# Themaister/Granite

Measured on AMD Instinct MI355X. Metric: Mpixels/s for clustered-light+post chain @4K; achieved HBM GB/s vs roofline, higher is better.
Workload: dtype f32

## Files before the change

### granite_amd/csrc/cluster.hip

```cpp
#include "ctx.hpp"
#include "device_common.hpp"
#include "device_vec.hpp"

namespace
{
__device__ __forceinline__ v4 mul_mat4(const float *m, v4 v)
{
	v4 r = mk4(m[0], m[1], m[2], m[3]) * v.x;
	r = r + mk4(m[4], m[5], m[6], m[7]) * v.y;
	r = r + mk4(m[8], m[9], m[10], m[11]) * v.z;
	r = r + mk4(m[12], m[13], m[14], m[15]) * v.w;
	return r;
}

__device__ __forceinline__ float min_tie2(float a, float b) { return a < b ? a : b; }
__device__ __forceinline__ float max_tie2(float a, float b) { return a > b ? a : b; }

struct TransformedSpot { v4 clip[5]; v4 z; };
struct CullSetup { v4 data[32]; };

__device__ __forceinline__ const gr_light_info *lights_of(const void *transforms)
{
	return reinterpret_cast<const gr_light_info *>(static_cast<const uint8_t *>(transforms) + GR_TRANSFORMS_OFFSET_LIGHTS);
}
// ... 111 lines not shown
	bool dual;
	switch (code)
	{
	case 1u: a = c0; b = c1; c = c2; dual = true; break;
	case 2u: a = c1; b = c2; c = c0; dual = true; break;
	case 4u: a = c2; b = c0; c = c1; dual = true; break;
	case 3u: a = c0; b = c1; c = c2; dual = false; break;
	case 5u: a = c2; b = c0; c = c1; dual = false; break;
	default: a = c1; b = c2; c = c0; dual = false; break;
	}
	const float target = 0.0f;
	if (dual)
	{
		const float l_ab = (target - a.z) / (b.z - a.z);
		const float l_ac = (target - a.z) / (c.z - a.z);
		const v3 ab = mix3(a, b, l_ab);
		const v3 ac = mix3(a, c, l_ac);
		emit_triangle(cs, num_triangles, Tri2{{xy(ab), xy(b), xy(ac)}}, cull);
		emit_triangle(cs, num_triangles, Tri2{{xy(ac), xy(b), xy(c)}}, cull);
	}
	else
	{
		const float la = (target - a.z) / (c.z - a.z);
		const float lb = (target - b.z) / (c.z - b.z);
		a = mix3(a, c, la);
		b = mix3(b, c, lb);
		emit_triangle(cs, num_triangles, Tri2{{xy(a), xy(b), xy(c)}}, cull);
	}
}

__device__ void clip_w_and_project(CullSetup &cs, uint32_t &num_triangles, v4 c0, v4 c1, v4 c2, float cull)
{
	const float MIN_W = 1.0f / 1024.0f;
	const uint32_t code = uint32_t(c0.w < MIN_W) + uint32_t(c1.w < MIN_W) * 2u + uint32_t(c2.w < MIN_W) * 4u;
	if (code == 7u)
		return;
	if (code == 0u)
	{
		clip_near_z(cs, num_triangles, Tri3{{xyz(c0) / c0.w, xyz(c1) / c1.w, xyz(c2) / c2.w}}, cull);
		return;
	}
	v4 a, b, c;
	bool dual;
	switch (code)
	{
	case 1u: a = c0; b = c1; c = c2; dual = true; break;
	case 2u: a = c1; b = c2; c = c0; dual = true; break;
	case 4u: a = c2; b = c0; c = c1; dual = true; break;
	case 3u: a = c0; b = c1; c = c2; dual = false; break;
	case 5u: a = c2; b = c0; c = c1; dual = false; break;
	default: a = c1; b = c2; c = c0; dual = false; break;
	}
	if (dual)
	{
		const float l_ab = (MIN_W - a.w) / (b.w - a.w);
		const float l_ac = (MIN_W - a.w) / (c.w - a.w);
		const v4 ab = mix4(a, b, l_ab);
		const v4 ac = mix4(a, c, l_ac);
		clip_near_z(cs, num_triangles, Tri3{{xyz(ab) / MIN_W, xyz(b) / b.w, xyz(ac) / MIN_W}}, cull);
		clip_near_z(cs, num_triangles, Tri3{{xyz(ac) / MIN_W, xyz(b) / b.w, xyz(c) / c.w}}, cull);
	}
	else
	{
		const float la = (MIN_W - a.w) / (c.w - a.w);
		const float lb = (MIN_W - b.w) / (c.w - b.w);
		a = mix4(a, c, la);
		b = mix4(b, c, lb);
		clip_near_z(cs, num_triangles, Tri3{{xyz(a) / MIN_W, xyz(b) / MIN_W, xyz(c) / c.w}}, cull);
	}
}

__device__ __forceinline__ void cluster_setup_of(bool point, const gr_light_info &li, const TransformedSpot &spot, CullSetup &cs,
                                                 const gr_cluster_params &params, const gr_push_cluster_setup &push)
{
	if (point)
	{
		const float radius = 1.0f / li.inv_radius;
		const v4 v4d = mul_mat4(push.view, mk4(li.position[0], li.position[1], li.position[2], 1.0f));
		const v3 view = mk3(v4d.x, -v4d.y, -v4d.z);
		const v2 r0 = project_sphere_flat(view.x, view.z, radius);
		const v2 r1 = project_sphere_flat(view.y, view.z, radius);
		const float xy_length = len2(mk2(view.x, view.y));
		v2 ct0, ct1;
		if (xy_length < 0.00001f)
		{
			ct0 = mk2(1.0f, 0.0f);
			ct1 = mk2(0.0f, 1.0f);
		}
		else
		{
			const float inv_xy_length = 1.0f / xy_length;
			ct0 = mk2(view.x, -view.y) * inv_xy_length;
			ct1 = mk2(view.y, view.x) * inv_xy_length;
		}
		const v2 txy = mk2(ct0.x * view.x + ct1.x * view.y, ct0.y * view.x + ct1.y * view.y);
		const v2 t0 = project_sphere_flat(txy.x, view.z, radius);
		const v2 t1 = project_sphere_flat(txy.y, view.z, radius);
		const bool ellipsis = !isinf(t0.x) && !isinf(t0.y) && !isinf(t1.x) && !isinf(t1.y);
		const v2 center = (mk2(t0.x, t1.x) + mk2(t0.y, t1.y)) * 0.5f;
		const v2 ellipse_radius = mk2(t0.y, t1.y) - center;
		cs.data[0] = mk4(r0.x * params.clip_scale[0], r1.x * params.clip_scale[1], r0.y * params.clip_scale[0],
		                 r1.y * params.clip_scale[1]);
		cs.data[1] = mk4(t0.x, t0.y, t1.x, t1.y);
		cs.data[2] = mk4(ct0.x, ct0.y, ct1.x, ct1.y);
		cs.data[3] = mk4(ellipsis ? 1.0f : 0.0f, 1.0f / ellipse_radius.x, 1.0f / ellipse_radius.y, 0.0f);
	}
	else
	{
		const v4 z = spot.z;
		if (z.x != 0.0f)
		{
			uint32_t n = 0u;
			const v4 c0 = spot.clip[0], c1 = spot.clip[1], c2 = spot.clip[2];
			const v4 c3 = spot.clip[3], c4 = spot.clip[4];
			clip_w_and_project(cs, n, c0, c1, c2, z.x);
			clip_w_and_project(cs, n, c0, c2, c3, z.x);
			clip_w_and_project(cs, n, c0, c3, c4, z.x);
			clip_w_and_project(cs, n, c0, c4, c1, z.x);
			clip_w_and_project(cs, n, c2, c1, c3, z.x);
			clip_w_and_project(cs, n, c4, c3, c1, z.x);
			cs.data[0].w = __uint_as_float(n);
		}
		else
			cs.data[0].w = __uint_as_float(0xffffffffu);
	}
}

__global__ __launch_bounds__(64) void k_cluster_setup(const void *transforms, const TransformedSpot *spots, CullSetup *setup,
                                                      gr_cluster_params params, gr_push_cluster_setup push)
{
	const uint32_t index = blockIdx.x * 64u + threadIdx.x;
	if (index >= push.num_lights)
		return;
	const bool point = (type_mask_of(transforms)[index >> 5u] & (1u << (index & 31u))) != 0u;
	cluster_setup_of(point, lights_of(transforms)[index], spots[index], setup[index], params, push);
}

__device__ bool test_point_light(const gr_cluster_params &prm, const CullSetup &cs, v2 uv, v2 uv_stride)
{
	const v4 eir = cs.data[3];
	if (eir.x != 0.0f)
	{
		const v4 tr = cs.data[1];
		const v4 ct = cs.data[2];
		const v2 center = (mk2(tr.x, tr.z) + mk2(tr.y, tr.w)) * 0.5f;
		const v2 cszw = mk2(prm.clip_scale[2], prm.clip_scale[3]);
		const v2 lo = uv * cszw;
		const v2 hi = (uv + uv_stride) * cszw;
		const v2 inv_r = mk2(eir.y, eir.z);
		const v2 d00 = (mk2(ct.x * lo.x + ct.z * lo.y, ct.y * lo.x + ct.w * lo.y) - center) * inv_r;
		const v2 d01 = (mk2(ct.x * lo.x + ct.z * hi.y, ct.y * lo.x + ct.w * hi.y) - center) * inv_r;
		const v2 d10 = (mk2(ct.x * hi.x + ct.z * lo.y, ct.y * hi.x + ct.w * lo.y) - center) * inv_r;
		const v2 d11 = (mk2(ct.x * hi.x + ct.z * hi.y, ct.y * hi.x + ct.w * hi.y) - center) * inv_r;
		const float max_diag = fmaxf(dist2(d00, d11), dist2(d01, d10));
		float min_sq_dist = 1.0f + max_diag;
		min_sq_dist *= min_sq_dist;
		return dot2(d00, d00) < min_sq_dist && dot2(d01, d01) < min_sq_dist && dot2(d10, d10) < min_sq_dist &&
		       dot2(d11, d11) < min_sq_dist;
	}
	const v4 bb = cs.data[0];
	const v2 hi = uv + uv_stride;
	return hi.x > bb.x && hi.y > bb.y && uv.x < bb.z && uv.y < bb.w;
}

__device__ bool test_spot_light(const CullSetup &cs, v2 uv, v2 uv_stride)
{
	const uint32_t num_triangles = __float_as_uint(cs.data[0].w);
	if (num_triangles > 8u)
		return true;
	const v2 hi = uv + uv_stride;
	for (uint32_t i = 0; i < num_triangles; i++)
	{
		const v4 bb = cs.data[4u * i + 3u];
		if (hi.x > bb.x && hi.y > bb.y && uv.x < bb.z && uv.y < bb.w)
		{
			v3 base = xyz(cs.data[4u * i]);
			const v3 dx = xyz(cs.data[4u * i + 1u]);
			const v3 dy = xyz(cs.data[4u * i + 2u]);
			base = base + dx * uv.x;
			base = base + dy * uv.y;
			base = base + mk3(dx.x > 0.0f ? uv_stride.x * dx.x : 0.0f, dx.y > 0.0f ? uv_stride.x * dx.y : 0.0f,
			                  dx.z > 0.0f ? uv_stride.x * dx.z : 0.0f);
			base = base + mk3(dy.x > 0.0f ? uv_stride.y * dy.x : 0.0f, dy.y > 0.0f ? uv_stride.y * dy.y : 0.0f,
			                  dy.z > 0.0f ? uv_stride.y * dy.z : 0.0f);
			if (base.x > 0.0f && base.y > 0.0f && base.z > 0.0f)
				return true;
		}
	}
	return false;
}

__global__ __launch_bounds__(64) void k_cluster_binning(const void *transforms, const CullSetup *setup, uint32_t *bitmask,
                                                        gr_cluster_params prm)
{
	const uint32_t lane = threadIdx.x;
	const uint32_t chunk = blockIdx.x;
	const uint32_t tile_x = blockIdx.y, tile_y = blockIdx.z;
	const v2 inv_res = mk2(prm.inv_resolution_xy[0], prm.inv_resolution_xy[1]);
	const uint32_t type_mask = type_mask_of(transforms)[chunk];

	const v2 tile_uv = mk2(2.0f * float(tile_x * 8u), 2.0f * float(tile_y * 8u)) * inv_res - mk2(1.0f, 1.0f);
	const v2 tile_stride = mk2(2.0f * 8.0f, 2.0f * 8.0f) * inv_res;

	bool passed = false;
	if (lane < 32u)
	{
		const uint32_t light_index = 32u * chunk + lane;
		if (light_index < uint32_t(prm.num_lights))
		{
			if ((type_mask >> lane) & 1u)
				passed = test_point_light(prm, setup[light_index], tile_uv, tile_stride);
			else
				passed = test_spot_light(setup[light_index], tile_uv, tile_stride);
		}
	}
	uint32_t ballot = uint32_t(__ballot(passed));

	const uint32_t px = tile_x * 8u + (lane & 7u), py = tile_y * 8u + (lane >> 3u);
	const v2 uv = mk2(2.0f * float(px), 2.0f * float(py)) * inv_res - mk2(1.0f, 1.0f);
	const v2 uv_stride = inv_res * 2.0f;
	uint32_t pixel_mask = 0u;
	while (ballot != 0u)
	{
		const int lsb = __builtin_ctz(ballot);
		ballot &= ballot - 1u;
		const uint32_t light_index = chunk * 32u + uint32_t(lsb);
		bool hit;
		if ((type_mask >> lsb) & 1u)
			hit = test_point_light(prm, setup[light_index], uv, uv_stride);
		else
			hit = test_spot_light(setup[light_index], uv, uv_stride);
		if (hit)
			pixel_mask |= 1u << lsb;
	}
	const uint32_t linear_coord = py * uint32_t(prm.resolution_xy[0]) + px;
	bitmask[size_t(linear_coord) * uint32_t(prm.num_lights_32) + chunk] = pixel_mask;
}

constexpr int ZR_THREADS = 256;
constexpr int ZR_SLICES_PER_WAVE = 4;
constexpr int ZR_SLICES = (ZR_THREADS / 64) * ZR_SLICES_PER_WAVE;

__device__ __forceinline__ uint32_t zr_wave_min(uint32_t v)
{
#pragma unroll
	for (int off = 32; off > 0; off >>= 1)
		v = min(v, uint32_t(__shfl_xor(int(v), off, 64)));
	return v;
}
__device__ __forceinline__ uint32_t zr_wave_max(uint32_t v)
{
#pragma unroll
	for (int off = 32; off > 0; off >>= 1)
		v = max(v, uint32_t(__shfl_xor(int(v), off, 64)));
	return v;
}

__device__ __forceinline__ void z_range_block(const uint2 *light_ranges, uint2 *out, const gr_push_z_range &push, uint32_t slice_block, uint8_t *smem,
                                              uint2 *copy_out)
{
	const uint32_t num_groups = (push.num_volumes + 63u) / 64u;
	uint2 *ranges = reinterpret_cast<uint2 *>(smem);
	uint2 *group_bounds = ranges + size_t(num_groups) * 64u;
	const uint32_t lane = threadIdx.x & 63u, wave = threadIdx.x >> 6u;

	for (uint32_t g = wave; g < num_groups; g += ZR_THREADS / 64)
	{
		const uint32_t i = g * 64u + lane;
		const uint2 r = i < push.num_volumes ? light_ranges[i] : make_uint2(0xffffffffu, 0u);
		ranges[i] = r;
		if (copy_out && i < push.num_volumes)
			copy_out[i] = r;
		const bool valid = r.x <= r.y;
		const uint32_t glo = zr_wave_min(valid ? r.x : 0xffffffffu), ghi = zr_wave_max(valid ? r.y : 0u);
		if (lane == 0)
			group_bounds[g] = make_uint2(glo, ghi);
	}
	__syncthreads();

	for (uint32_t s = 0; s < ZR_SLICES_PER_WAVE; s++)
	{
		const uint32_t z = slice_block * ZR_SLICES + wave * ZR_SLICES_PER_WAVE + s;
		if (z >= push.num_ranges)
			break;
		uint32_t first = 0xffffffffu, last = 0u;
		for (uint32_t base = 0; base < num_groups; base += 64u)
		{
			const uint32_t g = base + lane;
			const uint2 gb = g < num_groups ? group_bounds[g] : make_uint2(0xffffffffu, 0u);
			const uint64_t candidates = __ballot(gb.x <= z && z <= gb.y);
			if (first == 0xffffffffu)
			{
				uint64_t walk = candidates;
				while (walk != 0ull)
				{
					const uint32_t gg = base + uint32_t(__builtin_ctzll(walk));
					walk &= walk - 1ull;
					const uint2 r = ranges[gg * 64u + lane];
					const uint64_t m = __ballot(r.x <= z && z <= r.y);
					if (m != 0ull)
					{
						first = gg * 64u + uint32_t(__builtin_ctzll(m));
						break;
					}
				}
			}
			uint64_t walk = candidates;
			while (walk != 0ull)
			{
				const uint32_t top = 63u - uint32_t(__builtin_clzll(walk));
				walk &= ~(1ull << top);
				const uint32_t gg = base + top;
				const uint2 r = ranges[gg * 64u + lane];
				const uint64_t m = __ballot(r.x <= z && z <= r.y);
				if (m != 0ull)
				{
					last = max(last, gg * 64u + 63u - uint32_t(__builtin_clzll(m)));
					break;
				}
			}
		}
		if (lane == 0)
			out[z] = make_uint2(first, last);
	}
}

__global__ __launch_bounds__(ZR_THREADS) void k_cluster_z_range(const uint2 *light_ranges, uint2 *out, gr_push_z_range push)
{
	extern __shared__ __attribute__((aligned(16))) uint8_t smem[];
	z_range_block(light_ranges, out, push, blockIdx.x, smem, nullptr);
}

struct ClusterFrontArgs
{
	void *transforms;
	const gr_light_info *src_lights;
	const gr_mat_affine *src_models;
	const uint32_t *src_type_mask;
	TransformedSpot *spots;
	CullSetup *setup;
	gr_cluster_params params;
	gr_push_spot_transform spot_push;
	gr_push_cluster_setup setup_push;
	const uint2 *src_ranges;
	uint2 *light_ranges;
	uint2 *range_out;
	gr_push_z_range z_push;
	uint32_t light_blocks;
};

__global__ __launch_bounds__(ZR_THREADS) void k_cluster_front(ClusterFrontArgs a)
{
	extern __shared__ __attribute__((aligned(16))) uint8_t smem[];
	if (blockIdx.x >= a.light_blocks)
	{
		z_range_block(a.src_ranges, a.range_out, a.z_push, blockIdx.x - a.light_blocks, smem,
		              (blockIdx.x == a.light_blocks && a.light_ranges != a.src_ranges) ? a.light_ranges : nullptr);
		return;
	}
	const uint32_t index = blockIdx.x * ZR_THREADS + threadIdx.x;
	uint8_t *t = static_cast<uint8_t *>(a.transforms);
	uint32_t *dst_mask = reinterpret_cast<uint32_t *>(t + GR_TRANSFORMS_OFFSET_TYPE_MASK);
	if (a.src_type_mask != dst_mask && index < uint32_t(a.params.num_lights_32))
		dst_mask[index] = a.src_type_mask[index];
	if (index >= a.spot_push.num_lights)
		return;
	const gr_light_info li = a.src_lights[index];
	const gr_mat_affine m = a.src_models[index];
	gr_light_info *dst_lights = reinterpret_cast<gr_light_info *>(t + GR_TRANSFORMS_OFFSET_LIGHTS);
	gr_mat_affine *dst_models = reinterpret_cast<gr_mat_affine *>(t + GR_TRANSFORMS_OFFSET_MODEL);
	if (a.src_lights != dst_lights)
		dst_lights[index] = li;
	if (a.src_models != dst_models)
		dst_models[index] = m;
	const bool point = (a.src_type_mask[index >> 5u] & (1u << (index & 31u))) != 0u;
	const TransformedSpot spot = spot_transform_of(m, a.spot_push);
	a.spots[index] = spot;
	cluster_setup_of(point, li, spot, a.setup[index], a.params, a.setup_push);
}
}

extern "C" {

int gr_cluster_spot_transform(gr_ctx *ctx, gr_stream stream, const void *transforms, void *transformed_spots,
                              const gr_push_spot_transform *push)
{
	if (!ctx)
		return GR_ERR_INVALID_ARGUMENT;
	GR_CHECK_ARG(ctx, transforms && transformed_spots && push);
	GR_CHECK_ARG(ctx, push->num_lights <= GR_MAX_LIGHTS_BINDLESS);
	if (push->num_lights == 0)
		return GR_OK;
	gr_scoped_timing timing{ctx, gr_to_stream(stream), "cluster_spot_transform"};
	hipLaunchKernelGGL(k_spot_transform, dim3(gr_div_up(push->num_lights, 64)), dim3(64), 0, gr_to_stream(stream), transforms,
	                   static_cast<TransformedSpot *>(transformed_spots), *push);
	GR_CHECK_LAUNCH(ctx);
	return GR_OK;
}

int gr_cluster_setup(gr_ctx *ctx, gr_stream stream, const void *transforms, const void *transformed_spots, void *cull_setup,
                     const gr_cluster_params *params, const gr_push_cluster_setup *push)
{
	if (!ctx)
		return GR_ERR_INVALID_ARGUMENT;
	GR_CHECK_ARG(ctx, transforms && transformed_spots && cull_setup && params && push);
	GR_CHECK_ARG(ctx, push->num_lights <= GR_MAX_LIGHTS_BINDLESS);
	if (push->num_lights == 0)
		return GR_OK;
	gr_scoped_timing timing{ctx, gr_to_stream(stream), "cluster_setup"};
	hipLaunchKernelGGL(k_cluster_setup, dim3(gr_div_up(push->num_lights, 64)), dim3(64), 0, gr_to_stream(stream), transforms,
	                   static_cast<const TransformedSpot *>(transformed_spots), static_cast<CullSetup *>(cull_setup), *params,
	                   *push);
	GR_CHECK_LAUNCH(ctx);
	return GR_OK;
}

int gr_cluster_front(gr_ctx *ctx, gr_stream stream, const gr_cluster_front_args *args)
{
	if (!ctx)
		return GR_ERR_INVALID_ARGUMENT;
	GR_CHECK_ARG(ctx, args && args->transforms && args->transformed_spots && args->cull_setup && args->params && args->spot_push && args->setup_push);
	GR_CHECK_ARG(ctx, args->light_ranges && args->range_out && args->z_push);
	const uint32_t n = args->spot_push->num_lights;
	GR_CHECK_ARG(ctx, n >= 1 && n <= GR_MAX_LIGHTS_BINDLESS && n == args->setup_push->num_lights && int(n) == args->params->num_lights);
	GR_CHECK_ARG(ctx, args->z_push->num_volumes >= 1 && args->z_push->num_volumes <= GR_MAX_LIGHTS_BINDLESS && args->z_push->num_ranges > 0);
	uint8_t *t = static_cast<uint8_t *>(args->transforms);
	ClusterFrontArgs a = {};
	a.transforms = args->transforms;
	a.src_lights = args->src_lights ? static_cast<const gr_light_info *>(args->src_lights) : reinterpret_cast<const gr_light_info *>(t + GR_TRANSFORMS_OFFSET_LIGHTS);
	a.src_models = args->src_models ? static_cast<const gr_mat_affine *>(args->src_models) : reinterpret_cast<const gr_mat_affine *>(t + GR_TRANSFORMS_OFFSET_MODEL);
	a.src_type_mask = args->src_type_mask ? static_cast<const uint32_t *>(args->src_type_mask) : reinterpret_cast<const uint32_t *>(t + GR_TRANSFORMS_OFFSET_TYPE_MASK);
	a.spots = static_cast<TransformedSpot *>(args->transformed_spots);
	a.setup = static_cast<CullSetup *>(args->cull_setup);
	a.params = *args->params;
	a.spot_push = *args->spot_push;
	a.setup_push = *args->setup_push;
	a.light_ranges = reinterpret_cast<uint2 *>(args->light_ranges);
	a.src_ranges = args->src_ranges ? static_cast<const uint2 *>(args->src_ranges) : a.light_ranges;
	a.range_out = reinterpret_cast<uint2 *>(args->range_out);
	a.z_push = *args->z_push;
	a.light_blocks = gr_div_up(n, ZR_THREADS);
	const uint32_t num_groups = (a.z_push.num_volumes + 63u) / 64u;
	gr_scoped_timing timing{ctx, gr_to_stream(stream), "cluster_front"};
	hipLaunchKernelGGL(k_cluster_front, dim3(a.light_blocks + gr_div_up(a.z_push.num_ranges, ZR_SLICES)), dim3(ZR_THREADS),
	                   size_t(num_groups) * 65u * sizeof(uint2), gr_to_stream(stream), a);
	GR_CHECK_LAUNCH(ctx);
	return GR_OK;
}

int gr_cluster_binning(gr_ctx *ctx, gr_stream stream, const void *transforms, const void *cull_setup, uint32_t *bitmask,
                       const gr_cluster_params *params)
{
	if (!ctx)
		return GR_ERR_INVALID_ARGUMENT;
	GR_CHECK_ARG(ctx, transforms && cull_setup && bitmask && params);
	GR_CHECK_ARG(ctx, params->resolution_xy[0] > 0 && params->resolution_xy[1] > 0);
	GR_CHECK_ARG(ctx, (params->resolution_xy[0] & 7) == 0 && (params->resolution_xy[1] & 7) == 0);
	GR_CHECK_ARG(ctx, params->num_lights >= 0 && params->num_lights <= GR_MAX_LIGHTS_BINDLESS);
	GR_CHECK_ARG(ctx, params->num_lights_32 == (params->num_lights + 31) / 32);
	if (params->num_lights == 0)
		return GR_OK;
	dim3 grid(params->num_lights_32, params->resolution_xy[0] / 8, params->resolution_xy[1] / 8);
	gr_scoped_timing timing{ctx, gr_to_stream(stream), "cluster_binning"};
	hipLaunchKernelGGL(k_cluster_binning, grid, dim3(64), 0, gr_to_stream(stream), transforms,
	                   static_cast<const CullSetup *>(cull_setup), bitmask, *params);
	GR_CHECK_LAUNCH(ctx);
	return GR_OK;
}

int gr_cluster_z_range(gr_ctx *ctx, gr_stream stream, const uint32_t *light_ranges, uint32_t *out, const gr_push_z_range *push)
{
	if (!ctx)
		return GR_ERR_INVALID_ARGUMENT;
	GR_CHECK_ARG(ctx, light_ranges && out && push);
	GR_CHECK_ARG(ctx, push->num_volumes >= 1 && push->num_volumes <= GR_MAX_LIGHTS_BINDLESS);
	GR_CHECK_ARG(ctx, push->num_ranges > 0);
	gr_scoped_timing timing{ctx, gr_to_stream(stream), "cluster_z_range"};
	const uint32_t num_groups = (push->num_volumes + 63u) / 64u;
	hipLaunchKernelGGL(k_cluster_z_range, dim3(gr_div_up(push->num_ranges, ZR_SLICES)), dim3(ZR_THREADS),
	                   size_t(num_groups) * 65u * sizeof(uint2), gr_to_stream(stream), reinterpret_cast<const uint2 *>(light_ranges),
	                   reinterpret_cast<uint2 *>(out), *push);
	GR_CHECK_LAUNCH(ctx);
	return GR_OK;
}
}
```

### granite_amd/csrc/post.hip

```cpp
#include <cstdlib>
#include "ctx.hpp"
#include "device_common.hpp"

namespace
{
constexpr int POST_BLOCK_X = 32;
constexpr int POST_BLOCK_Y = 8;

#ifndef GR_POST_WAVE_PRIORITY
#define GR_POST_WAVE_PRIORITY 0
#endif
__device__ __forceinline__ void post_wave_priority()
{
	if (GR_POST_WAVE_PRIORITY != 0)
		__builtin_amdgcn_s_setprio(GR_POST_WAVE_PRIORITY);
}

template <bool DYNAMIC_EXPOSURE>
__global__ __launch_bounds__(POST_BLOCK_X *POST_BLOCK_Y) void k_bloom_threshold(DevImage hdr, DevImageRW out,
                                                                                const gr_luminance_data *lum,
                                                                                gr_push_bloom_threshold push, uint32_t y_first,
                                                                                uint32_t y_end, bool hdr_b10)
{
	post_wave_priority();
// ... 680 lines not shown

__device__ __forceinline__ void pyramid_publish(uint32_t *counter)
{
	__syncthreads();
	if (threadIdx.x == 0)
		__hip_atomic_fetch_add(counter, 1u, __ATOMIC_RELEASE, __HIP_MEMORY_SCOPE_AGENT);
}
__device__ __forceinline__ void pyramid_wait(uint32_t *counter, uint32_t target, uint32_t *giveups)
{
	if (threadIdx.x == 0)
	{
		uint32_t polls = 0;
		while (__hip_atomic_load(counter, __ATOMIC_RELAXED, __HIP_MEMORY_SCOPE_AGENT) < target)
		{
			__builtin_amdgcn_s_sleep(8);
			if (++polls == PYRAMID_SPIN_LIMIT)
			{
				__hip_atomic_fetch_add(giveups, 1u, __ATOMIC_RELAXED, __HIP_MEMORY_SCOPE_AGENT);
				break;
			}
		}
	}
	__syncthreads();
	__builtin_amdgcn_fence(__ATOMIC_ACQUIRE, "agent");
}

constexpr size_t PYRAMID_LDS_HEAD = sizeof(f16x4) * (HEAD_T_PATCH * HEAD_T_PATCH + HEAD_D0_PATCH * HEAD_D0_PATCH);
constexpr size_t PYRAMID_LDS_UP = sizeof(f16x4) * (UPALL_P2 * UPALL_P2 + UPALL_P1 * UPALL_P1) + sizeof(float) * (LUM_THREADS / 64);
constexpr size_t PYRAMID_LDS = PYRAMID_LDS_HEAD > PYRAMID_LDS_UP ? PYRAMID_LDS_HEAD : PYRAMID_LDS_UP;
static_assert(PYRAMID_LDS >= sizeof(f16x4) * TAIL_PATCH * TAIL_PATCH, "the down_pair patch fits too");
constexpr int PYRAMID_THREADS = 256;

template <bool DYNAMIC_EXPOSURE, bool D2_EXACT, bool D3_EXACT, bool U2_EXACT, bool U1_EXACT>
__global__ __launch_bounds__(PYRAMID_THREADS) void k_bloom_pyramid(PyramidArgs a)
{
	post_wave_priority();
	__shared__ __attribute__((aligned(16))) uint8_t s_raw[PYRAMID_LDS];
	const int thread = int(threadIdx.x);
	const uint32_t block = blockIdx.x;
	if (block < a.n0)
	{
		f16x4 *s_thr = reinterpret_cast<f16x4 *>(s_raw), *s_d0 = s_thr + HEAD_T_PATCH * HEAD_T_PATCH;
		down_head_block<DYNAMIC_EXPOSURE, PYRAMID_THREADS>(int(block % a.head_x), int(block / a.head_x), thread, s_thr, s_d0, a.hdr, a.thr, a.d0, a.d1, a.lum,
		                                                   a.inv_thr_w, a.inv_thr_h, a.hdr_b10);
		pyramid_publish(a.sync + 0);
	}
	else if (block < a.n0 + a.n1)
	{
		const uint32_t tile = block - a.n0;
		pyramid_wait(a.sync + 0, a.n0, a.sync + 3);
		down_pair_block<D2_EXACT, D3_EXACT, true, PYRAMID_THREADS>(int(tile % a.pair_x), int(tile / a.pair_x), thread, reinterpret_cast<f16x4 *>(s_raw), DevImage{a.d1.ptr, a.d1.w, a.d1.h, a.d1.pitch},
		                                                           a.d2, a.d3, a.history, a.push_d2, a.push_d3, 0u, uint32_t(a.d3.h));
		pyramid_publish(a.sync + 1);
	}
	else
	{
		const uint32_t tile = block - a.n0 - a.n1;
		pyramid_wait(a.sync + 1, a.n1, a.sync + 3);
		f16x4 *s_p2 = reinterpret_cast<f16x4 *>(s_raw), *s_p1 = s_p2 + UPALL_P2 * UPALL_P2;
		float *wave_partial = reinterpret_cast<float *>(s_p1 + UPALL_P1 * UPALL_P1);
		up_all_block<U2_EXACT, U1_EXACT, DYNAMIC_EXPOSURE, PYRAMID_THREADS>(int(tile % a.up_x), int(tile / a.up_x), thread, s_p2, s_p1, wave_partial,
		                                                                     DevImage{a.d3.ptr, a.d3.w, a.d3.h, a.d3.pitch}, a.u2, a.u1, a.u0, a.lum, a.push_u2, a.push_u1,
		                                                                     a.push_lum);
		__syncthreads();
		if (thread == 0 && __hip_atomic_fetch_add(a.sync + 2, 1u, __ATOMIC_ACQ_REL, __HIP_MEMORY_SCOPE_AGENT) == a.n2 - 1u)
		{
			__hip_atomic_store(a.sync + 0, 0u, __ATOMIC_RELAXED, __HIP_MEMORY_SCOPE_AGENT);
			__hip_atomic_store(a.sync + 1, 0u, __ATOMIC_RELAXED, __HIP_MEMORY_SCOPE_AGENT);
			__hip_atomic_store(a.sync + 2, 0u, __ATOMIC_RELEASE, __HIP_MEMORY_SCOPE_AGENT);
		}
	}
}

__device__ __forceinline__ float uncharted2_scaled(float x)
{
	constexpr float A = 0.15f, B = 0.50f, C = 0.10f, D = 0.20f, E = 0.02f, F = 0.30f, W = 11.2f;
	constexpr float white = ((W * (A * W + C * B) + D * E) / (W * (A * W + B) + D * F)) - E / F;
	constexpr float ws = 1.0f / white;
	const float num = fmaf(x, fmaf(A * ws, x, C * B * ws), D * E * ws);
	const float den = fmaf(x, fmaf(A, x, B), D * F);
	return fmaf(num, __builtin_amdgcn_rcpf(den), -(E / F) * ws);
}

constexpr int TONEMAP_PX = 4;
constexpr int TONEMAP_BLOCK_X = 64;
constexpr int TONEMAP_BLOCK_Y = 4;
constexpr int TONEMAP_ROW_GROUPS = 8;

template <int HALF>
__device__ __forceinline__ float mix_sub(uint32_t a, uint32_t b)
{
	float r;
	if (HALF)
		asm("v_fma_mix_f32 %0, %1, 1.0, -%2 op_sel:[1,0,1] op_sel_hi:[1,0,1]" : "=v"(r) : "v"(a), "v"(b));
	else
		asm("v_fma_mix_f32 %0, %1, 1.0, -%2 op_sel:[0,0,0] op_sel_hi:[1,0,1]" : "=v"(r) : "v"(a), "v"(b));
	return r;
}
template <int HALF>
__device__ __forceinline__ float mix_fma(float x, float y, uint32_t c)
{
	float r;
	if (HALF)
		asm("v_fma_mix_f32 %0, %1, %2, %3 op_sel:[0,0,1] op_sel_hi:[0,0,1]" : "=v"(r) : "v"(x), "v"(y), "v"(c));
	else
		asm("v_fma_mix_f32 %0, %1, %2, %3 op_sel:[0,0,0] op_sel_hi:[0,0,1]" : "=v"(r) : "v"(x), "v"(y), "v"(c));
	return r;
}
template <int HALF>
__device__ __forceinline__ float mix_add(uint32_t h, float b)
{
	float r;
	if (HALF)
		asm("v_fma_mix_f32 %0, %1, 1.0, %2 op_sel:[1,0,0] op_sel_hi:[1,0,0]" : "=v"(r) : "v"(h), "v"(b));
	else
		asm("v_fma_mix_f32 %0, %1, 1.0, %2 op_sel:[0,0,0] op_sel_hi:[1,0,0]" : "=v"(r) : "v"(h), "v"(b));
	return r;
}

constexpr uint32_t TONEMAP_TABLE_ROTATION = (TONEMAP_TABLE_MIN_BITS >> TONEMAP_TABLE_BUCKET_SHIFT) & 1023u;
static_assert(TONEMAP_TABLE_ENTRIES == 1025u && TONEMAP_TABLE_BUCKET_SHIFT == 17u, "bucket index = 10 bits of the float");
__device__ __forceinline__ uint32_t tonemap_srgb8_staged(float x, const uint2 *table)
{
	x = __builtin_amdgcn_fmed3f(x, 0x1p-12f, 0x1.fffffep+3f);
	const uint32_t offset = (__builtin_bit_cast(uint32_t, x) >> (TONEMAP_TABLE_BUCKET_SHIFT - 3u)) & (1023u << 3u);
	const uint2 e = *reinterpret_cast<const uint2 *>(reinterpret_cast<const uint8_t *>(table) + offset);
	return e.y + (x >= __builtin_bit_cast(float, e.x) ? 1u : 0u);
}

template <bool DYNAMIC_EXPOSURE, bool SRGB, bool QUARTER_BLOOM>
__global__ __launch_bounds__(TONEMAP_BLOCK_X *TONEMAP_BLOCK_Y) void k_tonemap(DevImage hdr, DevImage bloom, DevImageRW out,
                                                                              const gr_luminance_data *lum, const uint2 *encode_lut,
                                                                              gr_push_tonemap push, uint32_t y_first, uint32_t y_end, bool hdr_b10, int row_groups)
{
	post_wave_priority();
	__shared__ uint2 s_table[SRGB ? 1024 : 1];
	if (SRGB)
	{
		for (uint32_t i = threadIdx.y * TONEMAP_BLOCK_X + threadIdx.x; i < 1024u; i += TONEMAP_BLOCK_X * TONEMAP_BLOCK_Y)
		{
			const uint2 e = encode_lut[i];
			s_table[(i + TONEMAP_TABLE_ROTATION) & 1023u] = make_uint2(e.x, e.y | 0xff000000u);
		}
		__syncthreads();
	}
	const int x0 = (blockIdx.x * TONEMAP_BLOCK_X + threadIdx.x) * TONEMAP_PX;
	if (x0 >= hdr.w)
		return;
	float scale = push.dynamic_exposure;
	if (DYNAMIC_EXPOSURE)
		scale *= lum->average_inv_linear_luminance;
	const float inv_w = 1.0f / float(hdr.w), inv_h = 1.0f / float(hdr.h);

#pragma unroll 1
	for (int group = 0; group < row_groups; group++)
	{
		static_assert(TONEMAP_BLOCK_X == 64, "threadIdx.y is wave-uniform");
		const int y = __builtin_amdgcn_readfirstlane(int(y_first) + (blockIdx.y * row_groups + group) * TONEMAP_BLOCK_Y + int(threadIdx.y));
		if (uint32_t(y) >= y_end)
			return;
		const float v = (float(y) + 0.5f) * inv_h;

		const uint8_t *row = hdr.ptr + size_t(y) * hdr.pitch;
		uint32_t packed[TONEMAP_PX];
		const bool full = (x0 + TONEMAP_PX <= hdr.w) && ((reinterpret_cast<uintptr_t>(row) & 15u) == 0);
		u32x2 texels[TONEMAP_PX];
		if (hdr_b10)
		{
			uint32_t words[TONEMAP_PX];
			if (full)
			{
				const u32x4 t = *reinterpret_cast<const u32x4 *>(row + uint32_t(x0) * 4u);
				words[0] = t.x, words[1] = t.y, words[2] = t.z, words[3] = t.w;
			}
			else
			{
#pragma unroll
				for (int i = 0; i < TONEMAP_PX; i++)
					words[i] = *reinterpret_cast<const uint32_t *>(row + uint32_t(min(x0 + i, hdr.w - 1)) * 4u);
			}
#pragma unroll
			for (int i = 0; i < TONEMAP_PX; i++)
			{
				uint32_t rg, ba;
				expand_b10g11r11(words[i], rg, ba);
				texels[i] = u32x2{rg, ba};
			}
		}
		else if (full)
		{
			const u32x4 lo = *reinterpret_cast<const u32x4 *>(row + uint32_t(x0) * 8u);
			const u32x4 hi = *reinterpret_cast<const u32x4 *>(row + uint32_t(x0) * 8u + 16u);
			texels[0] = u32x2{lo.x, lo.y};
			texels[1] = u32x2{lo.z, lo.w};
			texels[2] = u32x2{hi.x, hi.y};
			texels[3] = u32x2{hi.z, hi.w};
		}
		else
		{
#pragma unroll
			for (int i = 0; i < TONEMAP_PX; i++)
				texels[i] = *reinterpret_cast<const u32x2 *>(row + uint32_t(min(x0 + i, hdr.w - 1)) * 8u);
		}

		float bloom_rgb[TONEMAP_PX][3];
		if (QUARTER_BLOOM)
		{
			const int k = x0 >> 2;
			const int j = (y >> 2) - (((y & 3) < 2) ? 1 : 0);
			const float wy = 0.125f + 0.25f * float((y + 2) & 3);
			const int r0 = clampi(j, 0, bloom.h - 1), r1 = clampi(j + 1, 0, bloom.h - 1);
			const uint8_t *row0 = bloom.ptr + size_t(r0) * bloom.pitch, *row1 = bloom.ptr + size_t(r1) * bloom.pitch;
			float col[3][3];
#pragma unroll
			for (int c = 0; c < 3; c++)
			{
				const uint32_t cx = uint32_t(clampi(k - 1 + c, 0, bloom.w - 1)) * 8u;
				const u32x2 t0 = *reinterpret_cast<const u32x2 *>(row0 + cx), t1 = *reinterpret_cast<const u32x2 *>(row1 + cx);
				col[c][0] = mix_fma<0>(mix_sub<0>(t1.x, t0.x), wy, t0.x);
				col[c][1] = mix_fma<1>(mix_sub<1>(t1.x, t0.x), wy, t0.x);
				col[c][2] = mix_fma<0>(mix_sub<0>(t1.y, t0.y), wy, t0.y);
			}
#pragma unroll
			for (int ch = 0; ch < 3; ch++)
			{
				bloom_rgb[0][ch] = fmaf(col[1][ch] - col[0][ch], 0.625f, col[0][ch]);
				bloom_rgb[1][ch] = fmaf(col[1][ch] - col[0][ch], 0.875f, col[0][ch]);
				bloom_rgb[2][ch] = fmaf(col[2][ch] - col[1][ch], 0.125f, col[1][ch]);
				bloom_rgb[3][ch] = fmaf(col[2][ch] - col[1][ch], 0.375f, col[1][ch]);
			}
		}
		else
		{
#pragma unroll
			for (int i = 0; i < TONEMAP_PX; i++)
			{
				const float u = (float(x0 + i) + 0.5f) * inv_w;
				const float4 b = sample_linear_rgba16f(bloom, u, v);
				bloom_rgb[i][0] = b.x;
				bloom_rgb[i][1] = b.y;
				bloom_rgb[i][2] = b.z;
			}
		}

		float x[TONEMAP_PX][3];
		uint32_t top = 0u;
#pragma unroll
		for (int i = 0; i < TONEMAP_PX; i++)
		{
			x[i][0] = mix_add<0>(texels[i].x, bloom_rgb[i][0]) * scale;
			x[i][1] = mix_add<1>(texels[i].x, bloom_rgb[i][1]) * scale;
			x[i][2] = mix_add<0>(texels[i].y, bloom_rgb[i][2]) * scale;
			if (SRGB)
				top = max(max(top, __builtin_bit_cast(uint32_t, x[i][0])), max(__builtin_bit_cast(uint32_t, x[i][1]), __builtin_bit_cast(uint32_t, x[i][2])));
		}
		if (SRGB && !__any(top >= 0x7f800000u))
		{
#pragma unroll
			for (int i = 0; i < TONEMAP_PX; i++)
				packed[i] = tonemap_srgb8_staged(x[i][0], s_table) | (tonemap_srgb8_staged(x[i][1], s_table) << 8) | (tonemap_srgb8_staged(x[i][2], s_table) << 16);
		}
		else
		{
#pragma unroll
			for (int i = 0; i < TONEMAP_PX; i++)
			{
				const float tr = uncharted2_scaled(x[i][0]), tg = uncharted2_scaled(x[i][1]), tb = uncharted2_scaled(x[i][2]);
				if (SRGB)
					packed[i] = encode_srgb8(tr) | (encode_srgb8(tg) << 8) | (encode_srgb8(tb) << 16) | 0xff000000u;
				else
					packed[i] = encode_unorm8(tr) | (encode_unorm8(tg) << 8) | (encode_unorm8(tb) << 16) | 0xff000000u;
			}
		}

		uint8_t *orow = out.ptr + size_t(y) * out.pitch;
		if (full && ((reinterpret_cast<uintptr_t>(orow) & 15u) == 0))
			*reinterpret_cast<u32x4 *>(orow + uint32_t(x0) * 4u) = u32x4{packed[0], packed[1], packed[2], packed[3]};
		else
		{
			for (int i = 0; i < TONEMAP_PX && x0 + i < hdr.w; i++)
				*reinterpret_cast<uint32_t *>(orow + uint32_t(x0 + i) * 4u) = packed[i];
		}
	}
}



static bool allow_stencil() { static const bool allow = gr_measurement_switch("GR_NO_STENCIL") == nullptr; return allow; }
static bool allow_tail_fusion() { static const bool allow = gr_measurement_switch("GR_NO_TAIL_FUSION") == nullptr; return allow; }

constexpr uint32_t RGBA16F = GR_FORMAT_R16G16B16A16_SFLOAT;
static bool same_size(const gr_image *a, const gr_image *b) { return a->width == b->width && a->height == b->height; }
static bool covers(const uint32_t threads[2], const gr_image *img) { return threads[0] == img->width && threads[1] == img->height; }
static bool is_reciprocal_of(const float inv[2], uint32_t width, uint32_t height) { return inv[0] == 1.0f / float(width) && inv[1] == 1.0f / float(height); }
static bool is_half_of(const gr_image *out, const gr_image *in) { return in->width == 2u * out->width && in->height == 2u * out->height; }
static bool down_patch_fits(const gr_image *fine, const gr_image *coarse)
{
	return float(fine->width) <= 2.3f * float(coarse->width) && float(fine->height) <= 2.3f * float(coarse->height);
}
static bool up_patch_fits(const gr_image *fine, const gr_image *coarse)
{
	return fine->width <= 2 * coarse->width && fine->height <= 2 * coarse->height && 2 * coarse->width <= fine->width + 1 && 2 * coarse->height <= fine->height + 1;
}
static bool has_texels(const gr_push_luminance *push) { return push->size[0] != 0 && push->size[1] != 0; }

static bool downsample_is_exact(const gr_image *in, const gr_push_bloom_downsample *push)
{
	return allow_stencil() && in->width == 2u * push->threads[0] && in->height == 2u * push->threads[1] && is_aligned(in, 16u) &&
	       is_reciprocal_of(push->inv_output_size, push->threads[0], push->threads[1]) && is_reciprocal_of(push->inv_input_size, in->width, in->height);
}
static bool upsample_is_exact(const gr_image *in, const gr_push_bloom_upsample *push)
{
	return allow_stencil() && push->threads[0] == 2u * in->width && push->threads[1] == 2u * in->height &&
	       is_reciprocal_of(push->inv_output_size, push->threads[0], push->threads[1]) && is_reciprocal_of(push->inv_input_size, in->width, in->height);
}
static bool threshold_is_exact(const gr_image *hdr, const gr_image *out, const gr_push_bloom_threshold *push)
{
	return allow_stencil() && hdr->width == 2u * push->threads[0] && hdr->height == 2u * push->threads[1] && (push->threads[0] & 1u) == 0 &&
	       out->width == push->threads[0] && is_aligned(hdr, 16u) && is_aligned(out, 16u) && is_reciprocal_of(push->inv_output_size, push->threads[0], push->threads[1]);
}

#define GR_RULE(cond) do { if (!(cond)) return #cond; } while (0)
#define GR_RULE_IMAGE(img, formats) do { if (gr_image_rule(img, formats)) return #img " is not a valid " #formats " image (image_args.hpp)"; } while (0)
#define GR_CHECK_FIT(ctx, fit) do { if (const char *rule__ = (fit)) return (ctx)->fail(GR_ERR_INVALID_ARGUMENT, "%s: invalid argument: %s", __func__, rule__); } while (0)

static const char *down_pair_fits(const gr_image *in, const gr_image *fine, const gr_image *coarse, const gr_push_bloom_downsample *push_fine,
                                  const gr_push_bloom_downsample *push_coarse)
{
	GR_RULE(push_fine != nullptr && push_coarse != nullptr);
	GR_RULE_IMAGE(in, RGBA16F);
	GR_RULE_IMAGE(fine, RGBA16F);
	GR_RULE_IMAGE(coarse, RGBA16F);
	GR_RULE(covers(push_fine->threads, fine) && covers(push_coarse->threads, coarse));
	GR_RULE(down_patch_fits(fine, coarse));
	return nullptr;
}

static const char *down_head_fits(const gr_image *hdr, const gr_image *threshold, const gr_image *d0, const gr_image *d1, const gr_push_bloom_threshold *push_t,
                                  const gr_push_bloom_downsample *push_d0, const gr_push_bloom_downsample *push_d1)
{
	GR_RULE(push_t && push_d0 && push_d1);
	GR_RULE_IMAGE(hdr, GR_HDR_FORMATS);
	GR_RULE_IMAGE(threshold, RGBA16F);
	GR_RULE_IMAGE(d0, RGBA16F);
	GR_RULE_IMAGE(d1, RGBA16F);
	GR_RULE(is_half_of(threshold, hdr) && is_half_of(d0, threshold) && is_half_of(d1, d0));
	GR_RULE(covers(push_t->threads, threshold) && push_d0->threads[0] == d0->width && push_d1->threads[0] == d1->width);
	GR_RULE(downsample_is_exact(threshold, push_d0) && downsample_is_exact(d0, push_d1));
	GR_RULE(is_aligned(hdr, 16u));
	return nullptr;
}

static const char *up_tail_fits(const gr_image *d3, const gr_image *u2, const gr_image *u1, const gr_push_bloom_upsample *push_u2,
                                const gr_push_bloom_upsample *push_u1)
{
	GR_RULE(push_u2 != nullptr && push_u1 != nullptr);
	GR_RULE_IMAGE(d3, RGBA16F);
	GR_RULE_IMAGE(u2, RGBA16F);
	GR_RULE_IMAGE(u1, RGBA16F);
	GR_RULE(covers(push_u2->threads, u2) && covers(push_u1->threads, u1));
	GR_RULE(up_patch_fits(u1, u2));
	return nullptr;
}

static const char *up_all_fits(const gr_image *d3, const gr_image *u2, const gr_image *u1, const gr_image *u0, const gr_push_bloom_upsample *push_u2,
                               const gr_push_bloom_upsample *push_u1, const gr_push_bloom_upsample *push_u0)
{
	GR_RULE(push_u0 != nullptr);
	if (const char *rule = up_tail_fits(d3, u2, u1, push_u2, push_u1))
		return rule;
	GR_RULE_IMAGE(u0, RGBA16F);
	GR_RULE(covers(push_u0->threads, u0) && upsample_is_exact(u1, push_u0));
	return nullptr;
}

static const char *luminance_fits(const gr_luminance_data *lum, const gr_push_luminance *push_lum)
{
	GR_RULE((lum == nullptr) == (push_lum == nullptr));
	GR_RULE(!push_lum || has_texels(push_lum));
	return nullptr;
}

static const char *pyramid_own_fits(const gr_bloom_pyramid_args *a)
{
	GR_RULE(same_size(&a->u2, &a->d2));
	GR_RULE_IMAGE(&a->history, RGBA16F);
	GR_RULE(same_size(&a->history, &a->d3) && !gr_images_overlap(&a->history, &a->d3));
	GR_RULE(!a->lum || has_texels(&a->push_luminance));
	return nullptr;
}

}

extern "C" {

int gr_bloom_threshold(gr_ctx *ctx, gr_stream stream, const gr_image *hdr, const gr_image *out, const gr_luminance_data *lum,
                       const gr_push_bloom_threshold *push)
{
	return gr_bloom_threshold_rows(ctx, stream, hdr, out, lum, push, nullptr);
}

int gr_bloom_threshold_rows(gr_ctx *ctx, gr_stream stream, const gr_image *hdr, const gr_image *out, const gr_luminance_data *lum,
                            const gr_push_bloom_threshold *push, const gr_rows *rows)
{
	if (!ctx)
		return GR_ERR_INVALID_ARGUMENT;
	GR_CHECK_ARG(ctx, push != nullptr);
	GR_CHECK_IMAGE(ctx, hdr, GR_HDR_FORMATS);
	GR_CHECK_IMAGE(ctx, out, RGBA16F);
	GR_CHECK_ARG(ctx, push->threads[0] <= out->width && push->threads[1] <= out->height);
	const bool b10 = hdr->format == GR_FORMAT_B10G11R11_UFLOAT_PACK32;
	if (push->threads[0] == 0 || push->threads[1] == 0)
		return GR_OK;
	const RowSpan span = resolve_rows(rows, push->threads[1]);
	if (span.count() == 0)
		return GR_OK;
	const bool exact = threshold_is_exact(hdr, out, push);
	const uint32_t pairs = push->threads[0] / 2u;
	dim3 block(POST_BLOCK_X, POST_BLOCK_Y);
	dim3 grid(gr_div_up(exact ? pairs : push->threads[0], POST_BLOCK_X), gr_div_up(span.count(), POST_BLOCK_Y));
	gr_scoped_timing timing{ctx, gr_to_stream(stream), "bloom_threshold"};
	with_flags(
	    [&](auto dynamic) {
		    if (exact)
			    hipLaunchKernelGGL(k_bloom_threshold_2to1<dynamic.value>, grid, block, 0, gr_to_stream(stream), to_dev(hdr), to_dev_rw(out), lum, pairs,
			                       push->inv_output_size[0], push->inv_output_size[1], span.first, span.end, b10);
		    else
			    hipLaunchKernelGGL(k_bloom_threshold<dynamic.value>, grid, block, 0, gr_to_stream(stream), to_dev(hdr), to_dev_rw(out), lum, *push, span.first,
// ... 351 lines not shown
```

Before: 41790.

## Bin two light chunks per wave and reuse bloom rows across tonemap groups

The cluster binning kernel now tests 64 lights per 64-lane wave, two 32-light chunks at once, instead of leaving half the lanes idle. It uses a 64-bit ballot and type mask and writes both mask words with one 8-byte store when alignment allows, halving the grid's x dimension. The tonemap kernel hoists row and bloom setup out of its row-group loop and carries the lower bloom row into the next group as the upper row, so each group loads one bloom row instead of two. This assumes consecutive groups advance exactly one quarter-res bloom row. The point-light diagonal distance is also recomputed with a single sqrt of the max squared length.

```diff
diff --git a/granite_amd/csrc/cluster.hip b/granite_amd/csrc/cluster.hip
--- a/granite_amd/csrc/cluster.hip
+++ b/granite_amd/csrc/cluster.hip
@@ -287,7 +287,8 @@
 		const v2 d01 = (mk2(ct.x * lo.x + ct.z * hi.y, ct.y * lo.x + ct.w * hi.y) - center) * inv_r;
 		const v2 d10 = (mk2(ct.x * hi.x + ct.z * lo.y, ct.y * hi.x + ct.w * lo.y) - center) * inv_r;
 		const v2 d11 = (mk2(ct.x * hi.x + ct.z * hi.y, ct.y * hi.x + ct.w * hi.y) - center) * inv_r;
-		const float max_diag = fmaxf(dist2(d00, d11), dist2(d01, d10));
+		const v2 e0 = d00 - d11, e1 = d01 - d10;
+		const float max_diag = sqrtf(fmaxf(dot2(e0, e0), dot2(e1, e1)));
 		float min_sq_dist = 1.0f + max_diag;
 		min_sq_dist *= min_sq_dist;
 		return dot2(d00, d00) < min_sq_dist && dot2(d01, d01) < min_sq_dist && dot2(d10, d10) < min_sq_dist &&
@@ -329,47 +330,58 @@
                                                         gr_cluster_params prm)
 {
 	const uint32_t lane = threadIdx.x;
-	const uint32_t chunk = blockIdx.x;
+	const uint32_t chunk0 = blockIdx.x * 2u, n32 = uint32_t(prm.num_lights_32);
+	const bool two_chunks = chunk0 + 1u < n32;
 	const uint32_t tile_x = blockIdx.y, tile_y = blockIdx.z;
 	const v2 inv_res = mk2(prm.inv_resolution_xy[0], prm.inv_resolution_xy[1]);
-	const uint32_t type_mask = type_mask_of(transforms)[chunk];
+	const uint32_t type_lo = type_mask_of(transforms)[chunk0], type_hi = two_chunks ? type_mask_of(transforms)[chunk0 + 1u] : 0u;
+	const uint64_t type_mask = uint64_t(type_lo) | (uint64_t(type_hi) << 32u);
 
 	const v2 tile_uv = mk2(2.0f * float(tile_x * 8u), 2.0f * float(tile_y * 8u)) * inv_res - mk2(1.0f, 1.0f);
 	const v2 tile_stride = mk2(2.0f * 8.0f, 2.0f * 8.0f) * inv_res;
 
 	bool passed = false;
-	if (lane < 32u)
-	{
-		const uint32_t light_index = 32u * chunk + lane;
+	{
+		const uint32_t light_index = 32u * chunk0 + lane;
 		if (light_index < uint32_t(prm.num_lights))
 		{
-			if ((type_mask >> lane) & 1u)
+			if ((type_mask >> lane) & 1ull)
 				passed = test_point_light(prm, setup[light_index], tile_uv, tile_stride);
 			else
 				passed = test_spot_light(setup[light_index], tile_uv, tile_stride);
 		}
 	}
-	uint32_t ballot = uint32_t(__ballot(passed));
+	uint64_t ballot = __ballot(passed);
 
 	const uint32_t px = tile_x * 8u + (lane & 7u), py = tile_y * 8u + (lane >> 3u);
 	const v2 uv = mk2(2.0f * float(px), 2.0f * float(py)) * inv_res - mk2(1.0f, 1.0f);
 	const v2 uv_stride = inv_res * 2.0f;
-	uint32_t pixel_mask = 0u;
-	while (ballot != 0u)
-	{
-		const int lsb = __builtin_ctz(ballot);
-		ballot &= ballot - 1u;
-		const uint32_t light_index = chunk * 32u + uint32_t(lsb);
+	uint32_t mask_lo = 0u, mask_hi = 0u;
+	while (ballot != 0ull)
+	{
+		const int lsb = __builtin_ctzll(ballot);
+		ballot &= ballot - 1ull;
+		const uint32_t light_index = chunk0 * 32u + uint32_t(lsb);
 		bool hit;
-		if ((type_mask >> lsb) & 1u)
+		if ((type_mask >> lsb) & 1ull)
 			hit = test_point_light(prm, setup[light_index], uv, uv_stride);
 		else
 			hit = test_spot_light(setup[light_index], uv, uv_stride);
-		if (hit)
-			pixel_mask |= 1u << lsb;
+		if (lsb < 32)
+			mask_lo |= hit ? 1u << lsb : 0u;
+		else
+			mask_hi |= hit ? 1u << (lsb - 32) : 0u;
 	}
 	const uint32_t linear_coord = py * uint32_t(prm.resolution_xy[0]) + px;
-	bitmask[size_t(linear_coord) * uint32_t(prm.num_lights_32) + chunk] = pixel_mask;
+	uint32_t *words = bitmask + (size_t(linear_coord) * n32 + chunk0);
+	if ((n32 & 1u) == 0u && (reinterpret_cast<uintptr_t>(bitmask) & 7u) == 0u)
+		*reinterpret_cast<uint2 *>(words) = make_uint2(mask_lo, mask_hi);
+	else
+	{
+		words[0] = mask_lo;
+		if (two_chunks)
+			words[1] = mask_hi;
+	}
 }
 
 constexpr int ZR_THREADS = 256;
@@ -595,7 +607,7 @@
 	GR_CHECK_ARG(ctx, params->num_lights_32 == (params->num_lights + 31) / 32);
 	if (params->num_lights == 0)
 		return GR_OK;
-	dim3 grid(params->num_lights_32, params->resolution_xy[0] / 8, params->resolution_xy[1] / 8);
+	dim3 grid(gr_div_up(uint32_t(params->num_lights_32), 2u), params->resolution_xy[0] / 8, params->resolution_xy[1] / 8);
 	gr_scoped_timing timing{ctx, gr_to_stream(stream), "cluster_binning"};
 	hipLaunchKernelGGL(k_cluster_binning, grid, dim3(64), 0, gr_to_stream(stream), transforms,
 	                   static_cast<const CullSetup *>(cull_setup), bitmask, *params);
diff --git a/granite_amd/csrc/post.hip b/granite_amd/csrc/post.hip
--- a/granite_amd/csrc/post.hip
+++ b/granite_amd/csrc/post.hip
@@ -856,16 +856,39 @@
 		scale *= lum->average_inv_linear_luminance;
 	const float inv_w = 1.0f / float(hdr.w), inv_h = 1.0f / float(hdr.h);
 
+	static_assert(TONEMAP_BLOCK_X == 64, "threadIdx.y is wave-uniform");
+	int y = __builtin_amdgcn_readfirstlane(int(y_first) + blockIdx.y * row_groups * TONEMAP_BLOCK_Y + int(threadIdx.y));
+	if (uint32_t(y) >= y_end)
+		return;
+	const uint8_t *row = hdr.ptr + size_t(y) * hdr.pitch;
+	uint8_t *orow = out.ptr + size_t(y) * out.pitch;
+
+	uint32_t cx[3] = {};
+	u32x2 upper[3] = {};
+	const uint8_t *below_row = nullptr;
+	int j = 0;
+	float wy = 0.0f;
+	if (QUARTER_BLOOM)
+	{
+		const int k = x0 >> 2;
+		j = (y >> 2) - (((y & 3) < 2) ? 1 : 0);
+		wy = 0.125f + 0.25f * float((y + 2) & 3);
+		const uint8_t *upper_row = bloom.ptr + size_t(clampi(j, 0, bloom.h - 1)) * bloom.pitch;
+		below_row = bloom.ptr + size_t(clampi(j + 1, 0, bloom.h - 1)) * bloom.pitch;
+#pragma unroll
+		for (int c = 0; c < 3; c++)
+		{
+			cx[c] = uint32_t(clampi(k - 1 + c, 0, bloom.w - 1)) * 8u;
+			upper[c] = *reinterpret_cast<const u32x2 *>(upper_row + cx[c]);
+		}
+	}
+
 #pragma unroll 1
-	for (int group = 0; group < row_groups; group++)
-	{
-		static_assert(TONEMAP_BLOCK_X == 64, "threadIdx.y is wave-uniform");
-		const int y = __builtin_amdgcn_readfirstlane(int(y_first) + (blockIdx.y * row_groups + group) * TONEMAP_BLOCK_Y + int(threadIdx.y));
+	for (int group = 0; group < row_groups; group++, y += TONEMAP_BLOCK_Y, row += size_t(hdr.pitch) * TONEMAP_BLOCK_Y, orow += size_t(out.pitch) * TONEMAP_BLOCK_Y)
+	{
 		if (uint32_t(y) >= y_end)
 			return;
-		const float v = (float(y) + 0.5f) * inv_h;
-
-		const uint8_t *row = hdr.ptr + size_t(y) * hdr.pitch;
+
 		uint32_t packed[TONEMAP_PX];
 		const bool full = (x0 + TONEMAP_PX <= hdr.w) && ((reinterpret_cast<uintptr_t>(row) & 15u) == 0);
 		u32x2 texels[TONEMAP_PX];
@@ -910,21 +933,19 @@
 		float bloom_rgb[TONEMAP_PX][3];
 		if (QUARTER_BLOOM)
 		{
-			const int k = x0 >> 2;
-			const int j = (y >> 2) - (((y & 3) < 2) ? 1 : 0);
-			const float wy = 0.125f + 0.25f * float((y + 2) & 3);
-			const int r0 = clampi(j, 0, bloom.h - 1), r1 = clampi(j + 1, 0, bloom.h - 1);
-			const uint8_t *row0 = bloom.ptr + size_t(r0) * bloom.pitch, *row1 = bloom.ptr + size_t(r1) * bloom.pitch;
 			float col[3][3];
 #pragma unroll
 			for (int c = 0; c < 3; c++)
 			{
-				const uint32_t cx = uint32_t(clampi(k - 1 + c, 0, bloom.w - 1)) * 8u;
-				const u32x2 t0 = *reinterpret_cast<const u32x2 *>(row0 + cx), t1 = *reinterpret_cast<const u32x2 *>(row1 + cx);
+				const u32x2 t0 = upper[c], t1 = *reinterpret_cast<const u32x2 *>(below_row + cx[c]);
 				col[c][0] = mix_fma<0>(mix_sub<0>(t1.x, t0.x), wy, t0.x);
 				col[c][1] = mix_fma<1>(mix_sub<1>(t1.x, t0.x), wy, t0.x);
 				col[c][2] = mix_fma<0>(mix_sub<0>(t1.y, t0.y), wy, t0.y);
+				upper[c] = t1;
 			}
+			j++;
+			if (j >= 0 && j + 1 < bloom.h)
+				below_row += bloom.pitch;
 #pragma unroll
 			for (int ch = 0; ch < 3; ch++)
 			{
@@ -936,6 +957,7 @@
 		}
 		else
 		{
+			const float v = (float(y) + 0.5f) * inv_h;
 #pragma unroll
 			for (int i = 0; i < TONEMAP_PX; i++)
 			{
@@ -977,7 +999,6 @@
 			}
 		}
 
-		uint8_t *orow = out.ptr + size_t(y) * out.pitch;
 		if (full && ((reinterpret_cast<uintptr_t>(orow) & 15u) == 0))
 			*reinterpret_cast<u32x4 *>(orow + uint32_t(x0) * 4u) = u32x4{packed[0], packed[1], packed[2], packed[3]};
 		else
```

Result: no change. 41970, median of 5 (+0.4%).
